# LucasAlegre/morl-baselines

Measured on NVIDIA H100. Metric: envelope_q_updates_per_sec, higher is better.
Workload: dtype f32

## Files before the change

morl_baselines_b200/csrc/gemm_planes.cu:

```cuda
#include <cuda.h>
#include <cuda_bf16.h>
#include <cuda_fp16.h>
#include <stdlib.h>
#include <string.h>

#include "common.cuh"
#include "gemm_tc.cuh"

namespace morl {

constexpr int kGemmBM = 128;
constexpr int kGemmThreads = 384;
constexpr int kGemmConsumerRegs = 232, kGemmProducerRegs = 40;
constexpr int kGemmBoxN = 32;

__device__ unsigned int g_plane_overflow;


__device__ __forceinline__ void note_overflow(float amax) {
    if (amax > 65504.f) atomicAdd(&g_plane_overflow, 1u);
}

#define MORL_DISPATCH_FMT(F_, ...)                                                         \
    switch (F_) {                                                                          \
// ... 323 lines not shown
            }
        }
    }
    if (!g.ln) return;
    const float inv_n = 1.0f / (float)N;
#pragma unroll
    for (int h = 0; h < 2; ++h) {
        float s = 0.f;
#pragma unroll
        for (int c = 0; c < 8; ++c)
            if (32 * c < N)
#pragma unroll
                for (int t = 0; t < 8; ++t) s = __fadd_rn(s, acc[16 * c + 4 * (t >> 1) + 2 * h + (t & 1)]);
        s = __fadd_rn(s, __shfl_xor_sync(0xffffffffu, s, 1));
        s = __fadd_rn(s, __shfl_xor_sync(0xffffffffu, s, 2));
        const float mean = __fmul_rn(s, inv_n);
        float v = 0.f;
#pragma unroll
        for (int c = 0; c < 8; ++c)
            if (32 * c < N)
#pragma unroll
                for (int t = 0; t < 8; ++t) {
                    const float d = __fsub_rn(acc[16 * c + 4 * (t >> 1) + 2 * h + (t & 1)], mean);
                    v = __fmaf_rn(d, d, v);
                }
        v = __fadd_rn(v, __shfl_xor_sync(0xffffffffu, v, 1));
        v = __fadd_rn(v, __shfl_xor_sync(0xffffffffu, v, 2));
        const float rstd = rsqrtf(__fadd_rn(__fmul_rn(v, inv_n), g.ln_eps));
#pragma unroll
        for (int c = 0; c < 8; ++c)
            if (32 * c < N)
#pragma unroll
                for (int t = 0; t < 8; ++t) {
                    const int col = 32 * c + 8 * (t >> 1) + 2 * l4 + (t & 1);
                    const int j = 16 * c + 4 * (t >> 1) + 2 * h + (t & 1);
                    const float gm = g.ln_gamma ? __ldg(g.ln_gamma + col) : 1.0f, bt = g.ln_beta ? __ldg(g.ln_beta + col) : 0.0f;
                    acc[j] = __fmaf_rn(__fmul_rn(__fsub_rn(acc[j], mean), rstd), gm, bt);
                }
    }
}

__device__ __forceinline__ void reload_bias(float* bias_s, const float* bias, int n_begin, int n_end, float mul) {
    bar_sync_named(1, 256);
    const int col = n_begin + (int)threadIdx.x;
    bias_s[threadIdx.x] = (bias && col < n_end) ? __ldg(bias + col) * mul : 0.f;
    bar_sync_named(1, 256);
}

template <int FMT, int SPLIT, bool PRE, typename AfterMma>
__device__ __forceinline__ void consume_unit(float (&acc)[128], const KSmem& s, Ring& ring, int n_kblk, int n_begin, int n_cnt, int rbase, int wg, int lane,
                                             long long* wait_cycles, AfterMma&& after_mma, const EpiArgs& e, const CUtensorMap* tmC, uint8_t* my_stage,
                                             uint32_t& n_stored, float& amax) {
#define MORL_UNIT(N_) \
    case N_: mma_unit<FMT, N_, SPLIT>(acc, s, ring, n_kblk, wg, lane, wait_cycles); break;
    switch (n_cnt) {
        MORL_UNIT(32) MORL_UNIT(64) MORL_UNIT(96) MORL_UNIT(128)
        default:
            if constexpr (!SPLIT) {
                switch (n_cnt) {
                    MORL_UNIT(160) MORL_UNIT(192) MORL_UNIT(224) MORL_UNIT(256)
                    default: __trap();
                }
            } else {
                __trap();
            }
    }
#undef MORL_UNIT
    after_mma();
#pragma unroll
    for (int c = 0; c < (SPLIT ? 4 : 8); ++c) {
        if (32 * c < n_cnt) {
            float a[16];
#pragma unroll
            for (int j = 0; j < 16; ++j) a[j] = SPLIT ? __fadd_rn(acc[16 * c + j], acc[64 + 16 * c + j]) : acc[16 * c + j];
            epilogue_chunk<FMT, PRE>(a, n_begin + 32 * c, rbase, lane, e, tmC, my_stage, n_stored, amax);
        }
    }
}

template <int FMT, int SPLIT, int EPI = kEpiPlain>
__global__ void __launch_bounds__(kGemmThreads, 1)
gemm_planes_kernel(const __grid_constant__ CUtensorMap tmA, const __grid_constant__ CUtensorMap tmB, const __grid_constant__ CUtensorMap tmC,
                   const GemmArgs g) {
    using L = KPlan<FMT>;
    extern __shared__ uint8_t gsmem_raw[];
    const KSmem s = carve_kplan<FMT>(gsmem_raw, (uint32_t)g.n_stages, g.b_stage);

    const int warp = threadIdx.x >> 5;
    const int lane = threadIdx.x & 31;
    const int BN = g.N_pad;
    const int n_tiles = (g.M + kGemmBM - 1) / kGemmBM;
    const int n_kblk = g.K / PlaneFmt<FMT>::BK;
    constexpr int kUnitN = SPLIT ? 128 : 256;
    const int col_units = (BN + kUnitN - 1) / kUnitN;
    const bool wide = BN > 256;
    const int n_work = n_tiles * col_units;
    auto unit_of = [&](int u, int& tile, int& n_begin, int& n_cnt) {
        tile = u / col_units;
        n_begin = (u - tile * col_units) * kUnitN;
        n_cnt = BN - n_begin < kUnitN ? BN - n_begin : kUnitN;
        if (g.reverse) tile = n_tiles - 1 - tile;
    };

    if (threadIdx.x == 0) {
        init_ring_barriers(s.full, s.empty, (uint32_t)g.n_stages);
        g_mbar_init_fence();
    }
    pdl_enter();
    for (int t = threadIdx.x; t < 256; t += blockDim.x) s.bias[t] = (g.bias && t < g.N) ? g.bias[t] : 0.f;
    __syncthreads();

    if (warp >= 8) {
        warpgroup_reg_dec<kGemmProducerRegs>();
        if (warp == 8 && lane == 0) {
            asm volatile("prefetch.tensormap [%0];" ::"l"(&tmA) : "memory");
            asm volatile("prefetch.tensormap [%0];" ::"l"(&tmB) : "memory");
            Ring ring((uint32_t)g.n_stages);
            long long w_empty = 0;
            for (int u = blockIdx.x; u < n_work; u += gridDim.x) {
                int tile, n_begin, n_cnt;
                unit_of(u, tile, n_begin, n_cnt);
                w_empty += load_unit<FMT>(s, ring, &tmA, &tmB, tile * kGemmBM, n_begin, n_cnt, n_kblk, g.stats != nullptr);
            }
            if (g.stats) atomicAdd(&g.stats[2], (unsigned long long)w_empty);
        }
    } else {
        warpgroup_reg_inc<kGemmConsumerRegs>();
        const int wg = warp >> 2;
        uint8_t* my_stage = s.c + warp * 2 * L::kStageC;
        uint32_t n_stored = 0;
        const float c_mul = ld_scale(g.c_scale);
        const bool folded = EPI == kEpiPlain && g.c_f32 == nullptr;
        const float fold = folded ? c_mul : 1.0f;
        if (warp == 0 && folded)
            for (int t = lane; t < 256; t += 32) s.bias[t] *= fold;
        bar_sync_named(1, 256);
        EpiArgs e;
        e.M = g.M; e.N = g.N;
        e.k_acc = fold / (ld_scale(g.a_scale) * ld_scale(g.b_scale));
        e.c_mul = folded ? 1.0f : c_mul;
        e.bias_s = s.bias; e.relu = g.relu; e.bits_in = g.bits_in; e.bits_out = g.bits_out; e.bits_ld = g.bits_ld; e.mask = g.mask;
        e.ld_mask = g.ld_mask; e.c_f32 = g.c_f32; e.ldc = g.ldc; e.planes = g.c_planes != nullptr; e.ldp = g.ldp;
        uint32_t key0 = 0, key1 = 0, ctr0 = 0;
        if constexpr (EPI == kEpiLn) {
            if (g.drop_seed) {
                const unsigned long long seed = *g.drop_seed;
                key0 = (uint32_t)seed;
                key1 = (uint32_t)(seed >> 32);
                ctr0 = *g.drop_offset;
            }
        }
        float amax = 0.f;
        float acc[128];
        Ring ring((uint32_t)g.n_stages);
        long long w_full = 0, busy = 0;
        const long long t_begin = g.stats ? clock64() : 0;
        for (int u = blockIdx.x; u < n_work; u += gridDim.x) {
            int tile, n_begin, n_cnt;
            unit_of(u, tile, n_begin, n_cnt);
            const int rbase = tile * kGemmBM + wg * 64 + (warp & 3) * 16;
            long long c1 = 0;
            consume_unit<FMT, SPLIT, EPI == kEpiLn>(acc, s, ring, n_kblk, n_begin, n_cnt, rbase, wg, lane, g.stats ? &w_full : nullptr, [&] {
                c1 = g.stats ? clock64() : 0;
                if (wide) {
                    reload_bias(s.bias, g.bias, n_begin, g.N, fold);
                    e.bias_s = s.bias - n_begin;
                }
                if constexpr (EPI == kEpiLn) ln_dropout_unit(acc, n_cnt, rbase, lane, s.bias, e.k_acc, g, key0, key1, ctr0);
            }, e, &tmC, my_stage, n_stored, amax);
            if (g.stats) busy += clock64() - c1;
        }
        if (g.stats && warp == 0 && lane == 0) {
            atomicAdd(&g.stats[0], (unsigned long long)w_full);
            atomicAdd(&g.stats[1], (unsigned long long)(clock64() - t_begin));
            atomicAdd(&g.stats[3], (unsigned long long)busy);
        }
        if (FMT == MORL_FMT_F16X2) note_overflow(amax);
        if (lane == 0) asm volatile("cp.async.bulk.wait_group 0;" ::: "memory");
    }
}

constexpr int kChainMaxJobs = 8;
constexpr int kChainLanes = 4;

struct alignas(64) ChainMaps {
    CUtensorMap A[kChainMaxJobs];
    CUtensorMap B[kChainMaxJobs];
    CUtensorMap C[kChainMaxJobs];
};

struct ChainArgs {
    int M, K;
    int k_first;
    int n_chains, n_layers;
    const float* bias[kChainMaxJobs];
    const float* b_scale[kChainMaxJobs];
    uint32_t* bits_out[kChainMaxJobs];
    const uint32_t* bits_in[kChainMaxJobs];
    const float* a_scale;
    int relu;
    int n_stages;
};

template <int FMT>
__global__ void __launch_bounds__(kGemmThreads, 1)
gemm_chain_kernel(const __grid_constant__ ChainMaps maps, const ChainArgs g) {
    using L = KPlan<FMT>;
    constexpr int BN = 256;
    extern __shared__ uint8_t gsmem_raw[];
    const KSmem s = carve_kplan<FMT>(gsmem_raw, (uint32_t)g.n_stages, L::kBStage);
    uint64_t* stored = s.empty + L::kMaxStages;

    const int warp = threadIdx.x >> 5;
    const int lane = threadIdx.x & 31;
    const int unit = blockIdx.x, n_units = gridDim.x;
    const int n_tiles = (g.M + kGemmBM - 1) / kGemmBM;
    const int n_kblk_full = g.K / PlaneFmt<FMT>::BK, n_kblk_first = g.k_first / PlaneFmt<FMT>::BK;
    const int tiles_per_group = kChainLanes / g.n_chains;
    const int cu0 = unit, cu1 = (unit + n_units / 2) % n_units;
    const int mt0 = cu0 < n_tiles ? (n_tiles - cu0 + n_units - 1) / n_units : 0;
    const int mt1 = g.n_chains > 1 ? (cu1 < n_tiles ? (n_tiles - cu1 + n_units - 1) / n_units : 0) : 0;
    const int n_groups = ((mt0 > mt1 ? mt0 : mt1) + tiles_per_group - 1) / tiles_per_group;
    auto unit_of = [&](int gi, int l, int ln, int& job, int& tile) {
        const int c = ln % g.n_chains, ti = gi * tiles_per_group + ln / g.n_chains;
        job = c * g.n_layers + l;
        tile = ti < (c ? mt1 : mt0) ? (c ? cu1 : cu0) + ti * n_units : -1;
    };

    if (threadIdx.x == 0) {
        init_ring_barriers(s.full, s.empty, (uint32_t)g.n_stages);
        for (int i = 0; i < kChainLanes; ++i) g_mbar_init(&stored[i], 8);
        g_mbar_init_fence();
    }
    pdl_enter();
    __syncthreads();

    if (warp >= 8) {
        warpgroup_reg_dec<kGemmProducerRegs>();
        if (warp == 8 && lane == 0) {
            Ring ring((uint32_t)g.n_stages);
            uint32_t done_on_lane[kChainLanes] = {0u, 0u, 0u, 0u};
            for (int gi = 0; gi < n_groups; ++gi)
                for (int l = 0; l < g.n_layers; ++l)
                    for (int ln = 0; ln < kChainLanes; ++ln) {
                        int job, tile;
                        unit_of(gi, l, ln, job, tile);
                        if (tile < 0) continue;
                        if (l > 0) {
                            g_mbar_wait(&stored[ln], (done_on_lane[ln] - 1u) & 1u);
                            asm volatile("fence.proxy.async.global;" ::: "memory");
                        }
                        ++done_on_lane[ln];
                        load_unit<FMT>(s, ring, &maps.A[job], &maps.B[job], tile * kGemmBM, 0, BN, l == 0 ? n_kblk_first : n_kblk_full, false);
                    }
        }
    } else {
        warpgroup_reg_inc<kGemmConsumerRegs>();
        const int wg = warp >> 2;
        uint8_t* my_stage = s.c + warp * 2 * L::kStageC;
        uint32_t n_stored = 0;
        const float s_act = ld_scale(g.a_scale);
        float amax = 0.f;
        float acc[128];
        Ring ring((uint32_t)g.n_stages);
        for (int gi = 0; gi < n_groups; ++gi)
            for (int l = 0; l < g.n_layers; ++l)
                for (int ln = 0; ln < kChainLanes; ++ln) {
                    int job, tile;
                    unit_of(gi, l, ln, job, tile);
                    if (tile < 0) continue;
                    reload_bias(s.bias, g.bias[job], 0, BN, s_act);
                    EpiArgs e;
                    e.M = g.M; e.N = BN;
                    e.k_acc = s_act / (s_act * ld_scale(g.b_scale[job]));
                    e.c_mul = 1.0f;
                    e.bias_s = s.bias; e.relu = g.relu; e.bits_in = g.bits_in[job]; e.bits_out = g.bits_out[job]; e.bits_ld = relu_bits_words(BN);
                    e.mask = nullptr; e.ld_mask = 0;
                    e.c_f32 = nullptr; e.ldc = 0; e.planes = 1; e.ldp = BN;
                    const int rbase = tile * kGemmBM + wg * 64 + (warp & 3) * 16;
                    consume_unit<FMT, 0, false>(acc, s, ring, l == 0 ? n_kblk_first : n_kblk_full, 0, BN, rbase, wg, lane, nullptr, [] {}, e,
                                                &maps.C[job], my_stage, n_stored, amax);
                    __syncwarp();
                    if (lane == 0) {
                        asm volatile("cp.async.bulk.wait_group 0;" ::: "memory");
                        g_mbar_arrive(&stored[ln]);
                    }
                }
        if (FMT == MORL_FMT_F16X2) note_overflow(amax);
    }
}

struct ResPlan {
    static constexpr int P = 2, BK = 32, kStages = 3;
    static constexpr uint32_t kRowB = BK * 2;
    static constexpr uint32_t kKBlock = P * kGemmBM * kRowB;
    static constexpr uint32_t kPlaneKB = kGemmBM * kRowB;
    static constexpr uint32_t kAct = 8 * kKBlock;
    static constexpr uint32_t kBStage = P * 256 * kRowB;
    static constexpr uint32_t kOffB = kAct;
    static constexpr uint32_t kOffBias = kOffB + kStages * kBStage;
    static constexpr uint32_t kOffBar = kOffBias + 1024;
    static constexpr uint32_t kBytes = kOffBar + 256 + 1024;
    static_assert(kBytes <= 232448, "dynamic shared memory of one CTA on sm_90 (227 KB)");
};

struct alignas(64) ResChainMaps {
    CUtensorMap A[2];
    CUtensorMap B[kChainMaxJobs];
    CUtensorMap C[kChainMaxJobs];
};

struct ResChainArgs {
    int M, K, k_first, n_chains, n_layers;
    const float* bias[kChainMaxJobs];
    const float* b_scale[kChainMaxJobs];
    uint32_t* bits_out[kChainMaxJobs];
    const uint32_t* bits_in[kChainMaxJobs];
    const float* a_scale;
    int relu;
    uint32_t store;
    const float* u[2];
    const float* v[2];
    int W;
    unsigned long long* stats;
};

__device__ __forceinline__ void mma_unit_resident(float (&acc)[128], uint32_t act, const KSmem& s, Ring& ring, int n_kblk, int wg, int lane,
                                                  long long* wait_cycles) {
    using F = PlaneFmt<MORL_FMT_F16X2>;
    using R = ResPlan;
    constexpr uint32_t b_plane = 256u * R::kRowB;
    const uint32_t a_wg = act + (uint32_t)wg * 64u * R::kRowB;
    uint32_t prev = 0;
    for (int kb = 0; kb < n_kblk; ++kb) {
        const long long c0 = wait_cycles ? clock64() : 0;
        g_mbar_wait(&s.full[ring.stage], ring.phase);
        if (wait_cycles) *wait_cycles += clock64() - c0;
        wgmma_fence();
        const uint32_t a0 = a_wg + (uint32_t)kb * R::kKBlock;
        const uint32_t b0 = g_smem_u32(s.b + ring.stage * R::kBStage);
#pragma unroll
        for (int ks = 0; ks < R::BK / 16; ++ks) {
#pragma unroll
            for (int t = 0; t < F::NPROD; ++t) {
                const uint64_t ad = make_desc_k<R::kRowB>(a0 + F::pa(t) * R::kPlaneKB + ks * 32);
                const uint64_t bd = make_desc_k<R::kRowB>(b0 + F::pb(t) * b_plane + ks * 32);
                Wgmma<256>::template mma<MORL_FMT_F16X2, 0, 0>(acc, ad, bd, (kb | ks | t) != 0 ? 1u : 0u);
            }
        }
        wgmma_commit();
        if (kb > 0) {
            wgmma_wait<1>();
            if (lane == 0) g_mbar_arrive(&s.empty[prev]);
        }
        prev = ring.stage;
        ring.advance();
    }
    wgmma_wait<0>();
    if (n_kblk > 0 && lane == 0) g_mbar_arrive(&s.empty[prev]);
}

__device__ __forceinline__ uint8_t* res_chunk(uint8_t* act, int kb, int row, int q) {
    return act + (uint32_t)kb * ResPlan::kKBlock + (uint32_t)row * ResPlan::kRowB + (uint32_t)((q ^ ((row >> 1) & 3)) << 4);
}

__global__ void __launch_bounds__(kGemmThreads, 1)
gemm_chain_resident_kernel(const __grid_constant__ ResChainMaps maps, const ResChainArgs g) {
    using F = PlaneFmt<MORL_FMT_F16X2>;
    using R = ResPlan;
    constexpr int P = R::P, BN = 256;
    extern __shared__ uint8_t gsmem_raw[];
    uint8_t* sm = align_1k(gsmem_raw);
    uint8_t* act = sm;
    KSmem s;
    s.a = nullptr;
    s.b = sm + R::kOffB;
    s.b_stage = R::kBStage;
    s.c = nullptr;
    s.bias = reinterpret_cast<float*>(sm + R::kOffBias);
    s.full = reinterpret_cast<uint64_t*>(sm + R::kOffBar);
    s.empty = s.full + R::kStages;
    uint64_t* act_full = s.empty + R::kStages;
    uint64_t* act_empty = act_full + 1;
    const bool pairs = g.u[0] != nullptr;

    const int warp = threadIdx.x >> 5;
    const int lane = threadIdx.x & 31;
    const int unit = blockIdx.x, n_units = gridDim.x;
    const int n_tiles = (g.M + kGemmBM - 1) / kGemmBM;
    const int n_kblk_full = g.K / R::BK, n_kblk_first = g.k_first / R::BK;
    const int cu0 = unit, cu1 = (unit + n_units / 2) % n_units;
    const int mt0 = cu0 < n_tiles ? (n_tiles - cu0 + n_units - 1) / n_units : 0;
    const int mt1 = g.n_chains > 1 ? (cu1 < n_tiles ? (n_tiles - cu1 + n_units - 1) / n_units : 0) : 0;
    const int n_ti = mt0 > mt1 ? mt0 : mt1;
    auto tile_row = [&](int ti, int c) { return ti < (c ? mt1 : mt0) ? ((c ? cu1 : cu0) + ti * n_units) * kGemmBM : -1; };

    if (threadIdx.x == 0) {
        init_ring_barriers(s.full, s.empty, R::kStages);
        g_mbar_init(act_full, 1);
        g_mbar_init(act_empty, 8);
        g_mbar_init_fence();
    }
    pdl_enter();
    __syncthreads();

    if (warp >= 8) {
        warpgroup_reg_dec<kGemmProducerRegs>();
        if (warp == 8 && lane == 0) {
            Ring ring((uint32_t)R::kStages);
            long long w_empty = 0;
            uint32_t n_in = 0;
            for (int ti = 0; ti < n_ti; ++ti)
                for (int c = 0; c < g.n_chains; ++c) {
                    const int row0 = tile_row(ti, c);
                    if (row0 < 0) continue;
                    for (int l = 0; l < g.n_layers; ++l) {
                        const int job = c * g.n_layers + l;
                        const int nkb = l == 0 ? n_kblk_first : n_kblk_full;
                        for (int kb = 0; kb < nkb; ++kb) {
                            if (!pairs && l == 0 && kb == (nkb < R::kStages ? nkb - 1 : R::kStages - 1)) {
                                if (n_in > 0) {
                                    const long long c0 = g.stats ? clock64() : 0;
                                    g_mbar_wait(act_empty, (n_in - 1u) & 1u);
                                    if (g.stats) w_empty += clock64() - c0;
                                }
                                g_mbar_expect_tx(act_full, (uint32_t)n_kblk_first * R::kKBlock);
                                for (int k = 0; k < n_kblk_first; ++k) tma_load_3d(act + k * R::kKBlock, &maps.A[c], act_full, k * R::BK, row0, 0);
                                ++n_in;
                            }
                            const long long c0 = g.stats ? clock64() : 0;
                            g_mbar_wait(&s.empty[ring.stage], ring.phase ^ 1u);
                            if (g.stats) w_empty += clock64() - c0;
                            uint64_t* full = &s.full[ring.stage];
                            g_mbar_expect_tx(full, R::kBStage);
                            uint8_t* bs = s.b + ring.stage * R::kBStage;
                            for (int p = 0; p < P; ++p) tma_load_3d(bs + (uint32_t)p * 256u * R::kRowB, &maps.B[job], full, kb * R::BK, 0, p);
                            ring.advance();
                        }
                    }
                }
            if (g.stats) atomicAdd(&g.stats[2], (unsigned long long)w_empty);
        }
    } else {
        warpgroup_reg_inc<kGemmConsumerRegs>();
        const int wg = warp >> 2, wr = warp & 3;
        const int l4 = lane & 3, lr = lane >> 2;
        const int trow = wg * 64 + wr * 16;
        const float s_act = ld_scale(g.a_scale);
        const uint32_t act_s = g_smem_u32(act);
        float amax = 0.f;
        float acc[128];
        Ring ring((uint32_t)R::kStages);
        long long w_full = 0, busy = 0, w_act = 0;
        const long long t_begin = g.stats ? clock64() : 0;
        uint32_t n_in = 0;
        for (int ti = 0; ti < n_ti; ++ti)
            for (int c = 0; c < g.n_chains; ++c) {
                const int row0 = tile_row(ti, c);
                if (row0 < 0) continue;
                if (pairs) {
                    if (lane == 0) asm volatile("cp.async.bulk.wait_group.read 0;" ::: "memory");
                    __syncwarp();
                    const float* u = c ? g.u[1] : g.u[0];
                    const float* v = c ? g.v[1] : g.v[0];
#pragma unroll
                    for (int h = 0; h < 2; ++h) {
                        const int rl = trow + lr + 8 * h, row = row0 + rl;
                        const bool ok = row < g.M;
                        const int b = ok ? row / g.W : 0, j = ok ? row - b * g.W : 0;
#pragma unroll 2
                        for (int kb = 0; kb < 8; ++kb) {
                            const int col = kb * 32 + 8 * l4;
                            uint32_t o[P][4];
                            if (ok) {
                                const float4* up = reinterpret_cast<const float4*>(u + (size_t)b * BN + col);
                                const float4* vp = reinterpret_cast<const float4*>(v + (size_t)j * BN + col);
                                const float4 u0 = __ldg(up), u1 = __ldg(up + 1), v0 = __ldg(vp), v1 = __ldg(vp + 1);
                                const float x[8] = {u0.x + v0.x, u0.y + v0.y, u0.z + v0.z, u0.w + v0.w, u1.x + v1.x, u1.y + v1.y, u1.z + v1.z, u1.w + v1.w};
#pragma unroll
                                for (int t = 0; t < 4; ++t) {
                                    uint32_t w[P];
                                    const float r0 = x[2 * t] < 0.f ? 0.f : x[2 * t], r1 = x[2 * t + 1] < 0.f ? 0.f : x[2 * t + 1];
                                    F::split2(r0 * s_act, r1 * s_act, w, amax);
#pragma unroll
                                    for (int p = 0; p < P; ++p) o[p][t] = w[p];
                                }
                            } else {
#pragma unroll
                                for (int t = 0; t < 4; ++t)
#pragma unroll
                                    for (int p = 0; p < P; ++p) o[p][t] = 0u;
                            }
                            uint8_t* dst = res_chunk(act, kb, rl, l4);
#pragma unroll
                            for (int p = 0; p < P; ++p) *reinterpret_cast<uint4*>(dst + p * R::kPlaneKB) = make_uint4(o[p][0], o[p][1], o[p][2], o[p][3]);
                        }
                    }
                    asm volatile("fence.proxy.async.shared::cta;" ::: "memory");
                    bar_sync_named(2 + wg, 128);
                }
                for (int l = 0; l < g.n_layers; ++l) {
                    const int job = c * g.n_layers + l;
                    const bool last = l == g.n_layers - 1, store = (g.store >> job) & 1u;
                    reload_bias(s.bias, g.bias[job], 0, BN, s_act);
                    if (!pairs && l == 0) {
                        const long long c0 = g.stats ? clock64() : 0;
                        g_mbar_wait(act_full, n_in & 1u);
                        if (g.stats) w_act += clock64() - c0;
                    }
                    mma_unit_resident(acc, act_s, s, ring, l == 0 ? n_kblk_first : n_kblk_full, wg, lane, g.stats ? &w_full : nullptr);
                    const long long c1 = g.stats ? clock64() : 0;
                    EpiArgs e;
                    e.M = g.M; e.N = BN;
                    e.k_acc = s_act / (s_act * ld_scale(g.b_scale[job]));
                    e.c_mul = 1.0f;
                    e.bias_s = s.bias; e.relu = g.relu; e.bits_in = g.bits_in[job]; e.bits_out = g.bits_out[job]; e.bits_ld = relu_bits_words(BN);
                    e.mask = nullptr; e.ld_mask = 0; e.c_f32 = nullptr; e.ldc = 0; e.planes = 1; e.ldp = BN;
                    const bool to_tile = !last || store;
                    if (to_tile) {
                        if (lane == 0) asm volatile("cp.async.bulk.wait_group.read 0;" ::: "memory");
                        __syncwarp();
                    }
                    const int rbase = row0 + trow;
#pragma unroll
                    for (int cc = 0; cc < 8; ++cc) {
                        float a[16];
#pragma unroll
                        for (int jj = 0; jj < 16; ++jj) a[jj] = acc[16 * cc + jj];
                        float x[2][8];
                        epilogue_values<false>(a, 32 * cc, rbase, lane, e, x);
                        if (to_tile) {
#pragma unroll
                            for (int h = 0; h < 2; ++h) {
                                const int rl = lr + 8 * h;
#pragma unroll
                                for (int q = 0; q < 4; ++q) {
                                    uint32_t w[P];
                                    F::split2(x[h][2 * q], x[h][2 * q + 1], w, amax);
                                    uint8_t* st = res_chunk(act, cc, trow + rl, q) + 4 * l4;
#pragma unroll
                                    for (int p = 0; p < P; ++p) *reinterpret_cast<uint32_t*>(st + p * R::kPlaneKB) = w[p];
                                }
                            }
                            if (store) {
                                asm volatile("fence.proxy.async.shared::cta;" ::: "memory");
                                __syncwarp();
                                if (lane == 0) {
                                    const uint32_t src = act_s + (uint32_t)cc * R::kKBlock + (uint32_t)trow * R::kRowB;
#pragma unroll
                                    for (int p = 0; p < P; ++p)
                                        asm volatile("cp.async.bulk.tensor.3d.global.shared::cta.bulk_group [%0, {%2, %3, %4}], [%1];" ::"l"(&maps.C[job]),
                                                     "r"(src + p * R::kPlaneKB), "r"(32 * cc), "r"(rbase), "r"(p)
                                                     : "memory");
                                    asm volatile("cp.async.bulk.commit_group;" ::: "memory");
                                }
                            }
                        }
                    }
                    if (!last) {
                        asm volatile("fence.proxy.async.shared::cta;" ::: "memory");
                        bar_sync_named(2 + wg, 128);
                    } else if (!pairs) {
                        __syncwarp();
                        if (lane == 0) {
                            asm volatile("cp.async.bulk.wait_group.read 0;" ::: "memory");
                            g_mbar_arrive(act_empty);
                        }
                    }
                    if (g.stats) busy += clock64() - c1;
                }
                ++n_in;
            }
        if (g.stats && warp == 0 && lane == 0) {
            atomicAdd(&g.stats[0], (unsigned long long)w_full);
            atomicAdd(&g.stats[1], (unsigned long long)(clock64() - t_begin));
            atomicAdd(&g.stats[3], (unsigned long long)busy);
            atomicAdd(&g.stats[4], (unsigned long long)w_act);
        }
        note_overflow(amax);
        if (lane == 0) asm volatile("cp.async.bulk.wait_group 0;" ::: "memory");
    }
}

constexpr int kMnKT = 32;

__device__ __forceinline__ uint64_t make_desc_mn_sw128(uint32_t smem_addr, uint32_t lbo_bytes) {
    uint64_t d = 0;
    d |= (uint64_t)((smem_addr >> 4) & 0x3FFF);
    d |= (uint64_t)((lbo_bytes >> 4) & 0x3FFF) << 16;
    d |= (uint64_t)(1024 >> 4) << 32;
    d |= (uint64_t)1 << 62;
    return d;
}

struct GemmMnArgs {
    int M;
    int n_tiles;
    int NB;
    int rows_per_split;
    float* partial;
    float* colsum_partial;
};

template <int FMT, int NB, bool COLSUM>
__device__ __forceinline__ void mma_mn_unit(const GemmMnArgs& g, int split, int row, int col0, uint8_t* smA, uint8_t* smB, uint32_t a_stage, uint32_t b_stage,
                                            uint32_t chunk_bytes, uint64_t ones_desc, int n_kblk, uint64_t* full, uint64_t* empty, int wg, int lane) {
    using F = PlaneFmt<FMT>;
    constexpr int P = F::P;
    constexpr uint32_t plane = kMnKT * 128u;
    float acc[NB / 2], cs[8];
#pragma unroll
    for (int i = 0; i < NB / 2; ++i) acc[i] = 0.f;
#pragma unroll
    for (int i = 0; i < 8; ++i) cs[i] = 0.f;
    uint32_t stage = 0, phase = 0, prev = 0;
    for (int kb = 0; kb < n_kblk; ++kb) {
        g_mbar_wait(&full[stage], phase);
        wgmma_fence();
        const uint32_t a0 = g_smem_u32(smA + stage * a_stage) + (uint32_t)wg * chunk_bytes;
        const uint32_t b0 = g_smem_u32(smB + stage * b_stage);
#pragma unroll
        for (int ks = 0; ks < kMnKT / 16; ++ks) {
#pragma unroll
            for (int t = 0; t < F::NPROD; ++t) {
                const uint64_t ad = make_desc_mn_sw128(a0 + F::pa(t) * plane + ks * 2048u, chunk_bytes);
                const uint64_t bd = make_desc_mn_sw128(b0 + F::pb(t) * plane + ks * 2048u, chunk_bytes);
                Wgmma<NB>::template mma<FMT, 1, 1>(acc, ad, bd, (kb | ks | t) != 0 ? 1u : 0u);
            }
            if constexpr (COLSUM) {
#pragma unroll
                for (int pl = P - 1; pl >= 0; --pl)
                    Wgmma<16>::template mma<FMT, 1, 1>(cs, make_desc_mn_sw128(a0 + pl * plane + ks * 2048u, chunk_bytes), ones_desc,
                                                       (kb | ks | (P - 1 - pl)) != 0 ? 1u : 0u);
            }
        }
        wgmma_commit();
        if (kb > 0) {
            wgmma_wait<1>();
            if (lane == 0) g_mbar_arrive(&empty[prev]);
        }
        prev = stage;
        if (++stage == (uint32_t)F::kStagesMn) {
            stage = 0;
            phase ^= 1u;
        }
    }
    wgmma_wait<0>();
    const int l4 = lane & 3;
#pragma unroll
    for (int h = 0; h < 2; ++h) {
        float* prow = g.partial + ((size_t)split * g.n_tiles * 128 + row + 8 * h) * g.NB + col0 + 2 * l4;
#pragma unroll
        for (int j = 0; j < NB / 8; ++j) *reinterpret_cast<float2*>(prow + 8 * j) = make_float2(acc[4 * j + 2 * h], acc[4 * j + 2 * h + 1]);
        if (COLSUM && l4 == 0) g.colsum_partial[(size_t)split * g.n_tiles * 128 + row + 8 * h] = cs[2 * h];
    }
}

template <int FMT>
__global__ void __launch_bounds__(kGemmThreads, 1)
gemm_planes_mn_kernel(const __grid_constant__ CUtensorMap tmA, const __grid_constant__ CUtensorMap tmB, const GemmMnArgs g) {
    using F = PlaneFmt<FMT>;
    constexpr int P = F::P;
    constexpr int kStages = F::kStagesMn;
    extern __shared__ uint8_t gsmem_raw[];
    uint8_t* gsmem = align_1k(gsmem_raw);
    constexpr uint32_t chunk_bytes = (uint32_t)P * kMnKT * 128u;
    constexpr uint32_t a_stage = 2u * chunk_bytes;
    constexpr uint32_t b_stage = 4u * chunk_bytes;
    const int k_units = g.NB > 256 ? 2 : 1;
    const int col0 = (int)(blockIdx.x / g.n_tiles % k_units) * 256;
    const int nb = g.NB - col0 < 256 ? g.NB - col0 : 256;
    const int nb_chunks = nb / 64;
    uint8_t* smA = gsmem;
    uint8_t* smB = gsmem + kStages * a_stage;
    uint64_t* full = reinterpret_cast<uint64_t*>(smB + kStages * b_stage);
    uint64_t* empty = full + kStages;
    uint8_t* ones_b = reinterpret_cast<uint8_t*>(empty + kStages);
    uint32_t* ones = reinterpret_cast<uint32_t*>(align_1k(ones_b));
    for (int t = threadIdx.x; t < 1024; t += blockDim.x) ones[t] = F::kOnes2;
    asm volatile("fence.proxy.async.shared::cta;" ::: "memory");

    const int warp = threadIdx.x >> 5, lane = threadIdx.x & 31;
    const int nt = blockIdx.x % g.n_tiles;
    const int split = blockIdx.x / (g.n_tiles * k_units);
    const int m_begin = split * g.rows_per_split;
    const int m_end = min(g.M, m_begin + g.rows_per_split);
    const int n_kblk = (m_end - m_begin + kMnKT - 1) / kMnKT;

    if (threadIdx.x == 0) {
        init_ring_barriers(full, empty, kStages);
        g_mbar_init_fence();
    }
    __syncthreads();
    pdl_enter();

    if (warp >= 8) {
        warpgroup_reg_dec<kGemmProducerRegs>();
        if (warp == 8 && lane == 0) {
            uint32_t stage = 0, phase = 0;
            for (int kb = 0; kb < n_kblk; ++kb) {
                g_mbar_wait(&empty[stage], phase ^ 1u);
                g_mbar_expect_tx(&full[stage], (2u + (uint32_t)nb_chunks) * chunk_bytes);
                const int m0 = m_begin + kb * kMnKT;
                for (int c = 0; c < 2; ++c) tma_load_3d(smA + stage * a_stage + c * chunk_bytes, &tmA, &full[stage], nt * 128 + c * 64, m0, 0);
                for (int c = 0; c < nb_chunks; ++c) tma_load_3d(smB + stage * b_stage + c * chunk_bytes, &tmB, &full[stage], col0 + c * 64, m0, 0);
                if (++stage == kStages) {
                    stage = 0;
                    phase ^= 1u;
                }
            }
        }
    } else {
        warpgroup_reg_inc<kGemmConsumerRegs>();
        const int wg = warp >> 2;
        const uint64_t ones_desc = make_desc_mn_sw128(g_smem_u32(ones), chunk_bytes);
        const bool colsum = g.colsum_partial != nullptr && col0 == 0;
        const int row = nt * 128 + wg * 64 + (warp & 3) * 16 + (lane >> 2);
#define MORL_UNIT(N_)                                                                                                                               \
    case N_:                                                                                                                                        \
        if (colsum) mma_mn_unit<FMT, N_, true>(g, split, row, col0, smA, smB, a_stage, b_stage, chunk_bytes, ones_desc, n_kblk, full, empty, wg, lane); \
        else mma_mn_unit<FMT, N_, false>(g, split, row, col0, smA, smB, a_stage, b_stage, chunk_bytes, ones_desc, n_kblk, full, empty, wg, lane);       \
        break;
        switch (nb) {
            MORL_UNIT(64) MORL_UNIT(128) MORL_UNIT(192) MORL_UNIT(256)
            default: __trap();
        }
#undef MORL_UNIT
    }
}

__global__ void __launch_bounds__(256) reduce_partials_kernel(const float* __restrict__ partial, int S, int prow, int pcol, int rows, int cols,
                                                              int transpose, float* __restrict__ out, int ld_out, int main_blocks,
                                                              const float* __restrict__ vec_partial, float* __restrict__ vec_out,
                                                              const float* __restrict__ scale_a, const float* __restrict__ scale_b) {
    pdl_enter();
    __shared__ float red[8][33];
    float mul = 1.0f / (ld_scale(scale_a) * ld_scale(scale_b));
    if ((int)blockIdx.x >= main_blocks) {
        partial = vec_partial;
        out = vec_out;
        pcol = 1; cols = 1; transpose = 0; ld_out = 1;
        mul = 1.0f / ld_scale(scale_a);
    }
    const int e = ((int)blockIdx.x >= main_blocks ? (int)blockIdx.x - main_blocks : (int)blockIdx.x) * 32 + threadIdx.x;
    const int total = rows * cols;
    float acc = 0.f;
    int r = 0, c = 0;
    if (e < total) {
        r = e / cols;
        c = e - r * cols;
        const float* p = partial + (size_t)r * pcol + c;
        const size_t stride = (size_t)prow * pcol;
        float a0 = 0.f, a1 = 0.f;
        int s = threadIdx.y;
        for (; s + 8 < S; s += 16) {
            a0 += p[(size_t)s * stride];
            a1 += p[(size_t)(s + 8) * stride];
        }
        if (s < S) a0 += p[(size_t)s * stride];
        acc = a0 + a1;
    }
    red[threadIdx.y][threadIdx.x] = acc;
    __syncthreads();
    if (threadIdx.y == 0 && e < total) {
        float t = red[0][threadIdx.x];
#pragma unroll
        for (int y = 1; y < 8; ++y) t += red[y][threadIdx.x];
        t *= mul;
        if (transpose)
            out[(size_t)c * ld_out + r] = t;
        else
            out[(size_t)r * ld_out + c] = t;
    }
}

__global__ void __launch_bounds__(256) reduce_partials_vec4_kernel(const float* __restrict__ partial, int S, int prow, int pcol, int rows, int cols,
                                                                   float* __restrict__ out, int ld_out, int main_blocks,
                                                                   const float* __restrict__ vec_partial, float* __restrict__ vec_out,
                                                                   const float* __restrict__ scale_a, const float* __restrict__ scale_b) {
    pdl_enter();
    __shared__ float4 red[8][33];
    if ((int)blockIdx.x >= main_blocks) {
        const float mul = 1.0f / ld_scale(scale_a);
        const int e = ((int)blockIdx.x - main_blocks) * 32 + threadIdx.x;
        float acc = 0.f;
        if (e < rows) {
            const float* p = vec_partial + e;
            float a0 = 0.f, a1 = 0.f;
            int s = threadIdx.y;
            for (; s + 8 < S; s += 16) {
                a0 += p[(size_t)s * prow];
                a1 += p[(size_t)(s + 8) * prow];
            }
            if (s < S) a0 += p[(size_t)s * prow];
            acc = a0 + a1;
        }
        red[threadIdx.y][threadIdx.x].x = acc;
        __syncthreads();
        if (threadIdx.y == 0 && e < rows) {
            float t = red[0][threadIdx.x].x;
#pragma unroll
            for (int y = 1; y < 8; ++y) t += red[y][threadIdx.x].x;
            vec_out[e] = t * mul;
        }
        return;
    }
    const float mul = 1.0f / (ld_scale(scale_a) * ld_scale(scale_b));
    const int e4 = ((int)blockIdx.x * 32 + threadIdx.x) * 4;
    const int total = rows * cols;
    float4 acc = make_float4(0.f, 0.f, 0.f, 0.f);
    int r = 0, c = 0;
    if (e4 < total) {
        r = e4 / cols;
// ... 1021 lines not shown
```

Before: 836.7.

## Split activation load barrier per k-block and batch pair-input loads

Replaces the single activation-full mbarrier with one barrier per k-block, so the first-layer MMA can start on early k-blocks while later activation tiles are still arriving through TMA. Separately, the pair-activation build loop now issues the u/v global loads for four k-blocks before doing the arithmetic, which raises memory-level parallelism. The cost is more barriers to initialise and wait on, and extra registers held by the batched loads inside a kernel that is already heavy on registers.

```diff
diff --git a/morl_baselines_b200/csrc/gemm_planes.cu b/morl_baselines_b200/csrc/gemm_planes.cu
--- a/morl_baselines_b200/csrc/gemm_planes.cu
+++ b/morl_baselines_b200/csrc/gemm_planes.cu
@@ -649,6 +649,7 @@
     static constexpr uint32_t kOffBar = kOffBias + 1024;
     static constexpr uint32_t kBytes = kOffBar + 256 + 1024;
     static_assert(kBytes <= 232448, "dynamic shared memory of one CTA on sm_90 (227 KB)");
+    static_assert((2 * kStages + 8 + 1) * 8 <= 256, "ring barriers, act_full[8] and act_empty fit in the barrier area");
 };
 
 struct alignas(64) ResChainMaps {
@@ -673,13 +674,18 @@
 };
 
 __device__ __forceinline__ void mma_unit_resident(float (&acc)[128], uint32_t act, const KSmem& s, Ring& ring, int n_kblk, int wg, int lane,
-                                                  long long* wait_cycles) {
+                                                  long long* wait_cycles, uint64_t* in_full, uint32_t in_parity, long long* in_cycles) {
     using F = PlaneFmt<MORL_FMT_F16X2>;
     using R = ResPlan;
     constexpr uint32_t b_plane = 256u * R::kRowB;
     const uint32_t a_wg = act + (uint32_t)wg * 64u * R::kRowB;
     uint32_t prev = 0;
     for (int kb = 0; kb < n_kblk; ++kb) {
+        if (in_full) {
+            const long long c0 = in_cycles ? clock64() : 0;
+            g_mbar_wait(&in_full[kb], in_parity);
+            if (in_cycles) *in_cycles += clock64() - c0;
+        }
         const long long c0 = wait_cycles ? clock64() : 0;
         g_mbar_wait(&s.full[ring.stage], ring.phase);
         if (wait_cycles) *wait_cycles += clock64() - c0;
@@ -728,7 +734,7 @@
     s.full = reinterpret_cast<uint64_t*>(sm + R::kOffBar);
     s.empty = s.full + R::kStages;
     uint64_t* act_full = s.empty + R::kStages;
-    uint64_t* act_empty = act_full + 1;
+    uint64_t* act_empty = act_full + 8;
     const bool pairs = g.u[0] != nullptr;
 
     const int warp = threadIdx.x >> 5;
@@ -744,7 +750,7 @@
 
     if (threadIdx.x == 0) {
         init_ring_barriers(s.full, s.empty, R::kStages);
-        g_mbar_init(act_full, 1);
+        for (int k = 0; k < 8; ++k) g_mbar_init(&act_full[k], 1);
         g_mbar_init(act_empty, 8);
         g_mbar_init_fence();
     }
@@ -771,8 +777,10 @@
                                     g_mbar_wait(act_empty, (n_in - 1u) & 1u);
                                     if (g.stats) w_empty += clock64() - c0;
                                 }
-                                g_mbar_expect_tx(act_full, (uint32_t)n_kblk_first * R::kKBlock);
-                                for (int k = 0; k < n_kblk_first; ++k) tma_load_3d(act + k * R::kKBlock, &maps.A[c], act_full, k * R::BK, row0, 0);
+                                for (int k = 0; k < n_kblk_first; ++k) {
+                                    g_mbar_expect_tx(&act_full[k], R::kKBlock);
+                                    tma_load_3d(act + k * R::kKBlock, &maps.A[c], &act_full[k], k * R::BK, row0, 0);
+                                }
                                 ++n_in;
                             }
                             const long long c0 = g.stats ? clock64() : 0;
@@ -815,14 +823,25 @@
                         const int rl = trow + lr + 8 * h, row = row0 + rl;
                         const bool ok = row < g.M;
                         const int b = ok ? row / g.W : 0, j = ok ? row - b * g.W : 0;
-#pragma unroll 2
-                        for (int kb = 0; kb < 8; ++kb) {
-                            const int col = kb * 32 + 8 * l4;
+#pragma unroll
+                        for (int k4 = 0; k4 < 8; k4 += 4) {
+                        float4 ua[4][2], va[4][2];
+#pragma unroll
+                        for (int i = 0; i < 4; ++i) {
+                            const int kb = k4 + i;
+                            const float4* up = reinterpret_cast<const float4*>(u + (size_t)b * BN + kb * 32 + 8 * l4);
+                            const float4* vp = reinterpret_cast<const float4*>(v + (size_t)j * BN + kb * 32 + 8 * l4);
+                            ua[i][0] = __ldg(up);
+                            ua[i][1] = __ldg(up + 1);
+                            va[i][0] = __ldg(vp);
+                            va[i][1] = __ldg(vp + 1);
+                        }
+#pragma unroll
+                        for (int i = 0; i < 4; ++i) {
+                            const int kb = k4 + i;
                             uint32_t o[P][4];
                             if (ok) {
-                                const float4* up = reinterpret_cast<const float4*>(u + (size_t)b * BN + col);
-                                const float4* vp = reinterpret_cast<const float4*>(v + (size_t)j * BN + col);
-                                const float4 u0 = __ldg(up), u1 = __ldg(up + 1), v0 = __ldg(vp), v1 = __ldg(vp + 1);
+                                const float4 u0 = ua[i][0], u1 = ua[i][1], v0 = va[i][0], v1 = va[i][1];
                                 const float x[8] = {u0.x + v0.x, u0.y + v0.y, u0.z + v0.z, u0.w + v0.w, u1.x + v1.x, u1.y + v1.y, u1.z + v1.z, u1.w + v1.w};
 #pragma unroll
                                 for (int t = 0; t < 4; ++t) {
@@ -841,6 +860,7 @@
                             uint8_t* dst = res_chunk(act, kb, rl, l4);
 #pragma unroll
                             for (int p = 0; p < P; ++p) *reinterpret_cast<uint4*>(dst + p * R::kPlaneKB) = make_uint4(o[p][0], o[p][1], o[p][2], o[p][3]);
+                        }
                         }
                     }
                     asm volatile("fence.proxy.async.shared::cta;" ::: "memory");
@@ -850,12 +870,8 @@
                     const int job = c * g.n_layers + l;
                     const bool last = l == g.n_layers - 1, store = (g.store >> job) & 1u;
                     reload_bias(s.bias, g.bias[job], 0, BN, s_act);
-                    if (!pairs && l == 0) {
-                        const long long c0 = g.stats ? clock64() : 0;
-                        g_mbar_wait(act_full, n_in & 1u);
-                        if (g.stats) w_act += clock64() - c0;
-                    }
-                    mma_unit_resident(acc, act_s, s, ring, l == 0 ? n_kblk_first : n_kblk_full, wg, lane, g.stats ? &w_full : nullptr);
+                    mma_unit_resident(acc, act_s, s, ring, l == 0 ? n_kblk_first : n_kblk_full, wg, lane, g.stats ? &w_full : nullptr,
+                                      !pairs && l == 0 ? act_full : nullptr, n_in & 1u, g.stats ? &w_act : nullptr);
                     const long long c1 = g.stats ? clock64() : 0;
                     EpiArgs e;
                     e.M = g.M; e.N = BN;
```

After: 840.9 (median of 6 runs). Within noise of the previous version (+0.5%).
